# Acciorocketships/mrs-gym

Hardware: NVIDIA B200
Metric: agent-steps/sec (higher is better)
Workload: dtype f32

## Files before the change

### include/mrs_b200.h

```cpp
#ifndef MRS_B200_H
#define MRS_B200_H

#include <stddef.h>

#ifdef __cplusplus
extern "C" {
#endif

#define MRS_ABI_VERSION 5
#define MRS_STATE_PLANES 13
#define MRS_CTRL_PLANES 18
#define MRS_STATS_SLOTS 8
#define MRS_SCRATCH_PLANES 7
#define MRS_SCRATCH_PAIR_SPLITS 32
#define MRS_SYNC_WORDS 8208
#define MRS_COMM_MAX_WORLD 16
#define MRS_COMM_HANDLE_BYTES 64

typedef enum {
    MRS_SET_TARGET_VEL = 0,
    MRS_SET_TARGET_POS = 1,
    MRS_SET_TARGET_ACCEL = 2,
    MRS_SET_FORCE = 3,
    MRS_SET_TARGET_ORI = 4,
    MRS_SET_CONTROL = 5,
    MRS_SET_SPEEDS = 6,
    MRS_NO_ACTION = 7
} MrsActionType;

typedef enum {
    MRS_X_NONE = 0,
    MRS_X_POS_VEL = 1,
    MRS_X_FULL = 2
} MrsStateLayout;

typedef enum {
    MRS_OK = 0,
    MRS_ERR_ARG = -1,
    MRS_ERR_CUDA = -2,
    MRS_ERR_UNSUPPORTED = -3
} MrsError;

#define MRS_STATUS_NAN_ACTION 1u
#define MRS_STATUS_NONFINITE 2u
#define MRS_STATUS_CONTACT_OVERFLOW 16u
#define MRS_STATUS_SYNC_TIMEOUT 8u
#define MRS_STATUS_COMM_TIMEOUT 4u
#define MRS_STATUS_NEIGHBOR_OVERFLOW 32u

#define MRS_STAT_AGENT_CONTACTS 0
#define MRS_STAT_GROUND_CONTACTS 1
#define MRS_STAT_NONFINITE 2
#define MRS_STAT_NAN_ACTIONS 3
#define MRS_STAT_CONTACT_CHUNKS 4
#define MRS_STAT_SOLVER_SWEEPS 5
#define MRS_STAT_NEIGHBOR_OVERFLOW 6

typedef struct {
    float mass, ixx, iyy, izz;
    float kf, km, arm;
    float gnd_eff_coeff, prop_radius, gnd_hclip;
    float drag_xy, drag_z;
    float dw1, dw2, dw3;
    float prop_x[4], prop_y[4];
    float pos_p, pos_i, pos_d;
    float vel_p, vel_i, vel_d;
    float ori_p[3], ori_i[3], ori_d[3];
    float min_pwm, max_pwm, pwm2rpm_a, pwm2rpm_b;
    float ctrl_dt, ctrl_gravity;
    float mix_ainv[16];
    float mix_a[16];
    float nnls_tab[16 * 16];
} MrsQuadParams;

typedef struct {
    float mass;
    float inertia[3];
    float lin_damping, ang_damping;
    float max_coord_vel;
    int gyro;
    float ang_motion_threshold;
    float erp2, slop, contact_margin;
    float mu_ground, ground_z;
    float col_radius, col_halfheight, col_margin;
    int ground_contact, agent_contact;
    float agent_radius;
    float contact_radius;
    float mu_agent;
    int solver_iters;
    float solver_tol;
} MrsPhysicsParams;

typedef struct {
    int E, N, K, L;
    int action_type;
    int state_layout;
    float dt, gravity;
    float comm_range;
// ... 106 lines not shown
```

### mrs-gym_b200/csrc/mrs_step.cuh

```cuda
#pragma once
#include "mrs_common.cuh"
#include "mrs_contact_env.cuh"

namespace mrs {


__device__ __forceinline__ float* plane_ptr(float* p0, unsigned S, int pl) {
    return reinterpret_cast<float*>(reinterpret_cast<char*>(p0) + (unsigned long long)S * (unsigned)(pl * 4));
}
__device__ __forceinline__ const float* plane_ptr(const float* p0, unsigned S, int pl) {
    return reinterpret_cast<const float*>(reinterpret_cast<const char*>(p0) + (unsigned long long)S * (unsigned)(pl * 4));
}

template <int MODE, int GT>
static __device__ __noinline__ void chunk_step_contact(const MrsConfig* cptr, const Derived* dptr, const MrsBuffers* bptr,
                                                       const StepArgs* aptr, int G_in, int chunk, int t0, int T, unsigned lane_mask,
                                                       float4* wpos, unsigned* sh_events) {
    const MrsConfig& c = *cptr;
    const Derived& d = *dptr;
    const MrsBuffers& b = *bptr;
    const StepArgs& a = *aptr;
    const int lane = threadIdx.x & 31;
    const int G = GT ? GT : G_in;
    const int N = GT ? GT : c.N, E = c.E;
// ... 87 lines not shown
                v[0] += dv[0]; v[1] += dv[1]; v[2] += dv[2];
                worst = fmaxf(worst, wr);
            }
        };
        for (int it = 0; it < cp.solver_iters; ++it) {
            worst = 0.f;
            if (alive && g.act) worst = ground_sweep(cp, g, lam_g, fl, v, wb);
            if constexpr (kStaticRounds) {
#pragma unroll
                for (int r = 0; r < kRoundsMax; ++r)
                    if ((ract >> r) & 1u) do_round(r, lam_p + 3 * r);
            } else {
                for (unsigned m = ract; m; m &= m - 1u) {
                    const int r = __ffs(m) - 1;
                    do_round(r, lam_p + 3 * r);
                }
            }
            if (alive) ++n_sweeps;
            for (int o = G >> 1; o > 0; o >>= 1) worst = fmaxf(worst, __shfl_xor_sync(kFull32, worst, o));
            alive = alive && !(worst < cp.solver_tol);
            if (!__any_sync(kFull32, alive)) break;
        }
        st.vx = v[0]; st.vy = v[1]; st.vz = v[2];
        st.wx = R[0] * wb[0] + R[1] * wb[1] + R[2] * wb[2];
        st.wy = R[3] * wb[0] + R[4] * wb[1] + R[5] * wb[2];
        st.wz = R[6] * wb[0] + R[7] * wb[1] + R[8] * wb[2];
        if ((lam_g[0] + lam_g[1]) + (lam_g[2] + lam_g[3]) > 0.f) ++n_ground;
        if constexpr (kStaticRounds) {
#pragma unroll
            for (int r = 0; r < kRoundsMax; ++r)
                if (((ract >> r) & 1u) && lam_p[3 * r] > 0.f) ++n_agent_rows;
        } else {
            for (unsigned m = ract; m; m &= m - 1u)
                if (lam_p[3 * (__ffs(m) - 1)] > 0.f) ++n_agent_rows;
        }
    }
    integrate(c, d, st);
    if (!agent_finite(st)) status |= MRS_STATUS_NONFINITE;
    if (a.X0 && mine) write_X(a.X0 - (long long)t * a.xstride, c.state_layout, s, st);
    if (a.A0) {
        float* Arow = a.A0 - (long long)t * a.astride + (size_t)s * N;
        __syncwarp();
        wpos[lane] = make_float4(st.px, st.py, st.pz, 0.f);
        __syncwarp();
        if (mine) {
            for (int j = 0; j < N; ++j) {
                const float4 pj = wpos[gb + j];
                const float hit = d.comm_inf ? 1.f : adjacency_pair(st.px, st.py, st.pz, pj.x, pj.y, pj.z, d.s_max);
                MRS_TAPE_ST(Arow + j, (j == ai) ? 0.f : hit);
            }
        }
        __syncwarp();
    }
    if (!mine) { status = 0; n_agent_rows = 0; n_ground = 0; n_sweeps = 0; }
    {
        const unsigned any_status = __reduce_or_sync(kFull32, status);
        const unsigned sum_rows = __reduce_add_sync(kFull32, n_agent_rows);
        const unsigned sum_gnd = __reduce_add_sync(kFull32, n_ground);
        const unsigned max_sw = __reduce_max_sync(kFull32, n_sweeps);
        if (lane == 0) {
            if (any_status) atomicOr(&sh_events[0], any_status);
            if (sum_rows) atomicAdd(&sh_events[1], sum_rows);
            if (sum_gnd) atomicAdd(&sh_events[2], sum_gnd);
            if (any_status & MRS_STATUS_NONFINITE) atomicAdd(&sh_events[3], 1u);
            if (any_status & MRS_STATUS_NAN_ACTION) atomicAdd(&sh_events[4], 1u);
            if (max_sw) atomicAdd(&sh_events[6], max_sw);
        }
    }
  }
    if (mine) {
        store_agent(b.state, S, s, st);
        store_ctrl<MODE>(b.ctrl, S, s, k);
    }
}

template <int MODE, int GT> __host__ __device__ constexpr int group_warp_smem_bytes() {
#ifdef MRS_EXP_OLDSMEM
    return 1024 + ((MRS_PREFETCH && GT != 0) ? mode_stage_floats<MODE>() * 4 : 0);
#else
    return 512 + ((MRS_PREFETCH && GT != 0) ? mode_stage_floats<MODE>() * 4 : 0);
#endif
}

constexpr int kSyncCount = 8, kSyncQueue = 16, kSyncQueueLen = 1024, kSyncQueues = 8;
#ifndef MRS_DEFAULT_CPS
#define MRS_DEFAULT_CPS 4
#endif
static_assert(kSyncQueue + kSyncQueues * kSyncQueueLen <= MRS_SYNC_WORDS, "sync buffer layout");

template <int MODE, int GT, int WPB, bool BAKED, bool MANY>
__global__ void __launch_bounds__(WPB * 32, WPB == 4 ? ModeTraits<MODE>::minb : (4 * ModeTraits<MODE>::minb) / WPB)
#ifdef MRS_EXP_NOGC
step_group_kernel(const __grid_constant__ MrsConfig c_in, const __grid_constant__ Derived d_in, const MrsBuffers b,
                  const StepArgs a) {
#else
step_group_kernel(const __grid_constant__ MrsConfig c_in, const __grid_constant__ Derived d_in,
                  const __grid_constant__ MrsBuffers b, const __grid_constant__ StepArgs a) {
#endif
    MrsConfig c_bk;
    Derived d_bk;
    if constexpr (BAKED) baked_fill(c_bk, d_bk, c_in, d_in);
    const MrsConfig& c = BAKED ? c_bk : c_in;
    const Derived& d = BAKED ? d_bk : d_in;
    extern __shared__ __align__(16) unsigned char smem_raw[];
    constexpr bool kFull = GT != 0;
    constexpr bool kStage = MRS_PREFETCH && kFull;
    constexpr int kWarpBytes = group_warp_smem_bytes<MODE, GT>();
    __shared__ int sh_counter, sh_hi, sh_range, sh_lo, sh_pull;
    __shared__ unsigned sh_epoch;
    __shared__ unsigned sh_events[7];
    const int lane = threadIdx.x & 31, wib = threadIdx.x >> 5;
    unsigned char* wbase = smem_raw + wib * kWarpBytes;
    float4* wpos = reinterpret_cast<float4*>(wbase);
#ifdef MRS_EXP_OLDSMEM
    float* stage = reinterpret_cast<float*>(wbase + 1024);
#else
    float* stage = reinterpret_cast<float*>(wbase + 512);
#endif
    const int G = GT ? GT : a.G;
    const int N = GT ? GT : c.N;
    const int E = c.E;
    const int gpw = 32 / G;
    const int ai = lane & (G - 1);
    const int gb = lane - ai;
    const unsigned S = (unsigned)E * (unsigned)N;
    const int wtotal = gridDim.x * WPB;
    const MrsPhysicsParams& ph = c.phys;
    const bool pair_contact = ph.agent_contact && N > 1;

    constexpr bool kLocal = WPB > 4;
    constexpr bool kHand = kLocal && MRS_PREFETCH && GT != 0 && !MANY;
    const int T = MANY ? a.T : 1;
    const int gw = blockIdx.x * WPB + wib;
    if (threadIdx.x < 7) sh_events[threadIdx.x] = 0u;
    if (threadIdx.x == 7) sh_pull = 0;
    const int role = kHand ? a.role : 0;
    if (role == 2) {
        asm volatile("griddepcontrol.launch_dependents;");
        if (threadIdx.x == 0) {
            const unsigned long long* q = b.sync + kSyncQueue + ((a.seq - 1) & (kSyncQueues - 1)) * kSyncQueueLen + blockIdx.x;
            const unsigned long long* q3 = b.sync + kSyncQueue + ((a.seq - 3) & (kSyncQueues - 1)) * kSyncQueueLen + (gridDim.x - 1);
#ifdef MRS_EXP_NOBOUND
            const bool bound = false;
#else
            const bool bound = a.seq >= 3;
#endif
            unsigned long long e = ld_acquire_gpu_u64(q), e3 = bound ? ld_acquire_gpu_u64(q3) : 0ull, t0 = 0;
            unsigned epoch = (unsigned)ld_acquire_gpu_u64(b.sync);
            auto pending = [&]() {
                const unsigned long long tag = (unsigned long long)epoch << 16;
                return (e >> 16) != (tag | (unsigned)a.seq) || (bound && (e3 >> 16) != (tag | (unsigned)(a.seq - 2)));
            };
            while (pending()) {
                if (t0 == 0) t0 = global_ns();
                else if (global_ns() - t0 > 2000000000ull) {
                    if (b.status) atomicOr(b.status, MRS_STATUS_SYNC_TIMEOUT);
                    asm volatile("griddepcontrol.wait;" ::: "memory");
                    e = blockIdx.x;
                    break;
                }
                e = ld_acquire_gpu_u64(q);
                if (bound) e3 = ld_acquire_gpu_u64(q3);
                epoch = (unsigned)ld_acquire_gpu_u64(b.sync);
            }
            if (blockIdx.x == 0) atomicExch(b.sync + kSyncCount + ((a.seq + 4) & (kSyncQueues - 1)), 0ull);
            sh_range = (int)(e & 0xffffull);
            sh_epoch = epoch;
        }
    } else {
        if (role == 0) asm volatile("griddepcontrol.launch_dependents;");
        asm volatile("griddepcontrol.wait;" ::: "memory");
        if (threadIdx.x == 0) sh_range = blockIdx.x;
        if (role == 1) {
            if (blockIdx.x == 0 && threadIdx.x == 0) {
#pragma unroll
                for (int q = 0; q < kSyncQueues; ++q) atomicExch(b.sync + kSyncCount + q, 0ull);
                atomicAdd(b.sync, 1ull);
                __threadfence();
            }
            __syncthreads();
            asm volatile("griddepcontrol.launch_dependents;");
        }
    }
    if (threadIdx.x == 0) {
        const int nwork = a.nchunks - a.chunk_lo;
        const int r = sh_range;
        sh_counter = sh_lo = a.chunk_lo + (int)(((long long)r * nwork) / gridDim.x);
        sh_hi = a.chunk_lo + (int)(((long long)(r + 1) * nwork) / gridDim.x);
    }
    unsigned* parked = reinterpret_cast<unsigned*>(smem_raw + WPB * kWarpBytes);
    for (int i = threadIdx.x; i < a.slow_slots; i += WPB * 32) parked[i] = 0xffffffffu;
    __syncthreads();
    auto draw = [&]() -> int {
        int v = 0;
        asm volatile("{\n .reg .pred p;\n elect.sync _|p, 0xffffffff;\n @p atom.shared.add.u32 %0, [%1], 1;\n}"
                     : "+r"(v) : "r"((unsigned)__cvta_generic_to_shared(&sh_counter)) : "memory");
        return v;
    };
    const int chunk_hi = sh_hi;
    auto claim = [&](int v) -> int { return (v < chunk_hi) ? v : -1; };
    constexpr int kNC = mode_nctrl<MODE>();
    constexpr int kA = ModeTraits<MODE>::A;
    constexpr int kActBeg = 96, kActEnd = kActBeg + 8 * kA;
    constexpr int kP12Beg = kActEnd, kP12End = kP12Beg + 8;
    constexpr int kCtlBeg = kP12End, kCtlEnd = kCtlBeg + 8 * kNC;
    constexpr int kPieces = kCtlEnd;
    static_assert(kPieces * 4 == mode_stage_floats<MODE>(), "stage layout");
    const unsigned lane_el = (unsigned)(lane >> 3) * S + (unsigned)(lane & 7) * 4u;
    auto prefetch = [&](int chunk) {
        const unsigned s0 = (unsigned)chunk * 32u;
#pragma unroll
        for (int i = 0; i < (kPieces + 31) / 32; ++i) {
            const int q = lane + 32 * i;
            const int lo = 32 * i, hi = 32 * i + 31;
            if (hi < kActBeg) {
                cp_async16(stage + 4 * q, b.state + (lane_el + s0 + (unsigned)(4 * i) * S));
            } else {
                if (lo < kActEnd && hi >= kActBeg && (lo >= kActBeg || q >= kActBeg) && (hi < kActEnd || q < kActEnd))
                    cp_async16(stage + 4 * q, a.actions + (s0 * (unsigned)kA + (unsigned)(q - kActBeg) * 4u));
                if (lo < kP12End && hi >= kP12Beg && (lo >= kP12Beg || q >= kP12Beg) && (hi < kP12End || q < kP12End))
                    cp_async16(stage + 4 * q, b.state + (12u * S + s0 + (unsigned)(q - kP12Beg) * 4u));
                if (kNC > 0 && lo < kCtlEnd && hi >= kCtlBeg && (lo >= kCtlBeg || q >= kCtlBeg) && (hi < kCtlEnd || q < kCtlEnd)) {
                    const int cq = q - kCtlBeg;
                    cp_async16(stage + 4 * q, b.ctrl + ((unsigned)mode_ctrl_plane<MODE>(cq >> 3) * S + s0 + (unsigned)(cq & 7) * 4u));
                }
            }
        }
        cp_async_commit();
    };
#ifdef MRS_TRACE
    unsigned long long* trace = reinterpret_cast<unsigned long long*>(b.scratch) + (size_t)gw * 8;
    unsigned long long* agg = reinterpret_cast<unsigned long long*>(b.scratch) + (size_t)8192 * 8 + (size_t)a.slot_x * 4;
    int trace_i = 0;
    auto stamp = [&]() {
        unsigned long long tns;
        asm volatile("mov.u64 %0, %%globaltimer;" : "=l"(tns));
        if (lane == 0 && trace_i < 8) trace[trace_i] = tns;
        if (threadIdx.x == 0 && trace_i == 0) atomicMin(agg + 0, tns);
        if (threadIdx.x == 0 && trace_i == 1) atomicMax(agg + 1, tns);
        ++trace_i;
    };
    auto stamp_end = [&]() {
        unsigned long long tns;
        asm volatile("mov.u64 %0, %%globaltimer;" : "=l"(tns));
        if (threadIdx.x == 0) { atomicMax(agg + 2, tns); atomicMin(agg + 3, tns); }
    };
    stamp();
#endif
#ifdef MRS_TRACE
    stamp();
#endif
    int chunk, chunk_next;
    if (kLocal) {
        chunk = claim(__shfl_sync(kFull32, draw(), 0));
        chunk_next = chunk >= 0 ? claim(__shfl_sync(kFull32, draw(), 0)) : -1;
    } else {
        chunk = a.chunk_lo + gw;
        chunk_next = chunk + wtotal;
        if (chunk >= a.nchunks) chunk = -1;
        if (chunk_next >= a.nchunks) chunk_next = -1;
    }
    if (kStage && chunk >= 0) prefetch(chunk);
    const int rounds_static = kLocal ? 0 : (a.nchunks - a.chunk_lo + wtotal - 1) / wtotal;
    int round_i = 0, my_parked = 0;
    while (chunk >= 0) {
        const int ticket = (kLocal && chunk_next >= 0) ? draw() : -1;
        const int e = chunk * gpw + (lane / G);
        const bool valid = kFull ? true : ((e < E) && (ai < N));
        const unsigned s = kFull ? (unsigned)chunk * 32u + (unsigned)lane
                                 : (valid ? (unsigned)e * (unsigned)N + (unsigned)ai : 0u);
        Agent st;
        Ctrl k;
        float4 act0 = make_float4(0.f, 0.f, 0.f, 0.f);
        if constexpr (kStage) {
            cp_async_wait_all();
            __syncwarp();
            st.px = stage[0 * 32 + lane]; st.py = stage[1 * 32 + lane]; st.pz = stage[2 * 32 + lane];
            st.qx = stage[3 * 32 + lane]; st.qy = stage[4 * 32 + lane]; st.qz = stage[5 * 32 + lane];
            st.qw = stage[6 * 32 + lane];
            st.vx = stage[7 * 32 + lane]; st.vy = stage[8 * 32 + lane]; st.vz = stage[9 * 32 + lane];
            st.wx = stage[10 * 32 + lane]; st.wy = stage[11 * 32 + lane]; st.wz = stage[4 * kP12Beg + lane];
            const float* cs = stage + 4 * kCtlBeg + lane;
            if constexpr (ModeTraits<MODE>::io) {
#pragma unroll
                for (int i = 0; i < 3; ++i) k.io[i] = cs[i * 32];
            }
            if constexpr (ModeTraits<MODE>::ip) {
#pragma unroll
                for (int i = 0; i < 3; ++i) k.ip[i] = cs[(3 + i) * 32];
            }
            if constexpr (ModeTraits<MODE>::vel) {
#pragma unroll
                for (int i = 0; i < 3; ++i) {
                    k.iv[i] = cs[(3 + i) * 32]; k.lve[i] = cs[(6 + i) * 32];
                    k.dve[i] = cs[(9 + i) * 32]; k.ltv[i] = cs[(12 + i) * 32];
                }
            }
            const float* as = stage + 4 * kActBeg + kA * lane;
            if constexpr (kA == 4) act0 = *reinterpret_cast<const float4*>(as);
            if constexpr (kA == 3) act0 = make_float4(as[0], as[1], as[2], 0.f);
            __syncwarp();
            if (chunk_next >= 0) prefetch(chunk_next);
        } else if (valid) {
            load_agent(b.state, S, s, st);
            load_ctrl<MODE>(b.ctrl, S, s, k);
        } else {
            dummy_agent(st);
#pragma unroll
            for (int i = 0; i < 3; ++i) k.io[i] = k.ip[i] = k.iv[i] = k.lve[i] = k.dve[i] = k.ltv[i] = 0.f;
        }
        float* Xs = a.X0;
        float* As = a.A0;
        if (!kStage) {
            float tmp[4] = {0.f, 0.f, 0.f, 0.f};
            if (valid) (void)load_action<MODE>(a.actions, (size_t)s, tmp);
            act0 = make_float4(tmp[0], tmp[1], tmp[2], tmp[3]);
        }
        bool state_stored = false;
        for (int t = 0; t < T; ++t, Xs -= a.xstride, As -= a.astride) {
            unsigned status = 0;
            unsigned n_agent_rows = 0, n_ground = 0;
            float rpm[4];
            float act[4] = {act0.x, act0.y, act0.z, act0.w};
            if (kA > 0 && valid && (isnan(act0.x) || isnan(act0.y) || isnan(act0.z) || (kA == 4 && isnan(act0.w))))
                status |= MRS_STATUS_NAN_ACTION;
            if (MANY && t + 1 < T && valid) {
                float tmp[4];
                (void)load_action<MODE>(a.actions, (size_t)(t + 1) * S + s, tmp);
                act0 = make_float4(tmp[0], tmp[1], tmp[2], tmp[3]);
            }

#ifdef MRS_EXP_COPYONLY
            st.px += act[0] * 1e-12f;
            if (false) {
#else
            {
#endif
            float dw = 0.f;
// ... 103 lines not shown
                            MRS_TAPE_ST(reinterpret_cast<float4*>(Arow0 + col), make_float4(v0[0], v0[1], v0[2], v0[3]));
                            MRS_TAPE_ST(reinterpret_cast<float4*>(Arow0 + GT + col), make_float4(v1[0], v1[1], v1[2], v1[3]));
                        }
                    } else if (valid) {
                        for (int j = 0; j < N; ++j) Arow[j] = (j == ai) ? 0.f : 1.f;
                    }
                } else {
                    __syncwarp();
                    wpos[lane] = make_float4(st.px, st.py, st.pz, 0.f);
                    __syncwarp();
                    if constexpr (GT != 0) {
                        const int h = lane & 1;
                        const float4 r0 = wpos[lane & ~1], r1 = wpos[lane | 1];
                        float* Arow0 = As + (size_t)(s & ~1u) * GT;
                        const int d0 = (ai & ~1) - 4 * h;
#pragma unroll
                        for (int qq = 0; qq < GT / 8; ++qq) {
                            const int col = 8 * qq + 4 * h;
                            float4 pj[4];
#pragma unroll
                            for (int u = 0; u < 4; ++u) pj[u] = wpos[gb + col + u];
                            float v0[4], v1[4];
#pragma unroll
                            for (int u = 0; u < 4; ++u) {
                                const float h0 = adjacency_pair(r0.x, r0.y, r0.z, pj[u].x, pj[u].y, pj[u].z, d.s_max);
                                const float h1 = adjacency_pair(r1.x, r1.y, r1.z, pj[u].x, pj[u].y, pj[u].z, d.s_max);
                                v0[u] = (8 * qq + u == d0) ? 0.f : h0;
                                v1[u] = (8 * qq + u == d0 + 1) ? 0.f : h1;
                            }
                            MRS_TAPE_ST(reinterpret_cast<float4*>(Arow0 + col), make_float4(v0[0], v0[1], v0[2], v0[3]));
                            MRS_TAPE_ST(reinterpret_cast<float4*>(Arow0 + GT + col), make_float4(v1[0], v1[1], v1[2], v1[3]));
                        }
                    } else if (valid) {
                        if ((N & 3) == 0) {
#pragma unroll 2
                            for (int j = 0; j < N; j += 4) {
                                float4 pj[4];
#pragma unroll
                                for (int u = 0; u < 4; ++u) pj[u] = wpos[gb + j + u];
                                float v[4];
#pragma unroll
                                for (int u = 0; u < 4; ++u) {
                                    const float hit = adjacency_pair(st.px, st.py, st.pz, pj[u].x, pj[u].y, pj[u].z, d.s_max);
                                    v[u] = (j + u == ai) ? 0.f : hit;
                                }
                                MRS_TAPE_ST(reinterpret_cast<float4*>(Arow + j), make_float4(v[0], v[1], v[2], v[3]));
                            }
                        } else {
                            for (int j = 0; j < N; ++j) {
                                const float4 pj = wpos[gb + j];
                                const float hit = adjacency_pair(st.px, st.py, st.pz, pj.x, pj.y, pj.z, d.s_max);
                                Arow[j] = (j == ai) ? 0.f : hit;
                            }
                        }
                    }
                }
            }
            }
            if (!valid || state_stored) { status = 0; n_agent_rows = 0; n_ground = 0; }
            if (__reduce_or_sync(kFull32, status | n_agent_rows | n_ground)) {
                const unsigned any_status = __reduce_or_sync(kFull32, status);
                const unsigned sum_rows = __reduce_add_sync(kFull32, n_agent_rows);
                const unsigned sum_gnd = __reduce_add_sync(kFull32, n_ground);
                if (lane == 0) {
                    if (any_status) atomicOr(&sh_events[0], any_status);
                    if (sum_rows) atomicAdd(&sh_events[1], sum_rows);
                    if (sum_gnd) atomicAdd(&sh_events[2], sum_gnd);
                    if (any_status & MRS_STATUS_NONFINITE) atomicAdd(&sh_events[3], 1u);
                    if (any_status & MRS_STATUS_NAN_ACTION) atomicAdd(&sh_events[4], 1u);
                }
            }
        }

        if (valid && !state_stored) {
            float* p0 = b.state + s;
            *plane_ptr(p0, S, 0) = st.px; *plane_ptr(p0, S, 1) = st.py; *plane_ptr(p0, S, 2) = st.pz;
            *plane_ptr(p0, S, 3) = st.qx; *plane_ptr(p0, S, 4) = st.qy; *plane_ptr(p0, S, 5) = st.qz;
            *plane_ptr(p0, S, 6) = st.qw;
            *plane_ptr(p0, S, 7) = st.vx; *plane_ptr(p0, S, 8) = st.vy; *plane_ptr(p0, S, 9) = st.vz;
            *plane_ptr(p0, S, 10) = st.wx; *plane_ptr(p0, S, 11) = st.wy; *plane_ptr(p0, S, 12) = st.wz;
            store_ctrl<MODE>(b.ctrl, S, s, k);
        }
#ifdef MRS_TRACE
        stamp();
#endif
        chunk = chunk_next;
        ++round_i;
        if (kLocal) {
            chunk_next = (chunk >= 0) ? claim(__shfl_sync(kFull32, ticket, 0)) : -1;
        } else {
            chunk_next = (chunk >= 0 && chunk + wtotal < a.nchunks) ? chunk + wtotal : -1;
        }
    }
#ifndef MRS_EXP_NOCALL
    if (__syncthreads_or(my_parked)) {
        const int n_slots = kLocal ? sh_hi - sh_lo : WPB * rounds_static;
        for (;;) {
            int i = 0;
            if (lane == 0) i = atomicAdd(&sh_pull, 1);
            i = __shfl_sync(kFull32, i, 0);
            if (i >= n_slots) break;
            const unsigned e = parked[i];
            if (e == 0xffffffffu) continue;
            const int w = (int)(e >> 16);
            const int pc = kLocal ? sh_lo + i : a.chunk_lo + blockIdx.x * WPB + w + (i - w * rounds_static) * wtotal;
            chunk_step_contact<MODE, GT>(&c_in, &d_in, &b, &a, GT ? GT : a.G, pc, (int)(e & 0xffffu), T, kFull32, wpos, sh_events);
        }
    }
#endif
    __syncthreads();
    if (threadIdx.x == 0) {
        if (sh_events[0] && b.status) atomicOr(b.status, sh_events[0]);
        if (b.stats) {
            if (sh_events[1]) atomicAdd(b.stats + MRS_STAT_AGENT_CONTACTS, (unsigned long long)sh_events[1]);
            if (sh_events[2]) atomicAdd(b.stats + MRS_STAT_GROUND_CONTACTS, (unsigned long long)sh_events[2]);
            if (sh_events[3]) atomicAdd(b.stats + MRS_STAT_NONFINITE, (unsigned long long)sh_events[3]);
            if (sh_events[4]) atomicAdd(b.stats + MRS_STAT_NAN_ACTIONS, (unsigned long long)sh_events[4]);
            if (sh_events[5]) atomicAdd(b.stats + MRS_STAT_CONTACT_CHUNKS, (unsigned long long)sh_events[5]);
            if (sh_events[6]) atomicAdd(b.stats + MRS_STAT_SOLVER_SWEEPS, (unsigned long long)sh_events[6]);
        }
        if (role != 0) {
            __threadfence();
            const unsigned epoch = (role == 1) ? (unsigned)ld_acquire_gpu_u64(b.sync) : sh_epoch;
            const int q = a.seq & (kSyncQueues - 1);
            const unsigned long long j = atomicAdd(b.sync + kSyncCount + q, 1ull);
            st_release_gpu_u64(b.sync + kSyncQueue + q * kSyncQueueLen + (int)(j & (kSyncQueueLen - 1)),
                               ((unsigned long long)epoch << 32) | ((unsigned long long)(a.seq + 1) << 16) | (unsigned)sh_range);
        }
    }
#ifdef MRS_TRACE
    stamp_end();
#endif
}

template <int LPA>
__device__ __forceinline__ float group_sum(float v) {
#pragma unroll
    for (int o = LPA / 2; o > 0; o >>= 1) v += __shfl_xor_sync(kFull32, v, o);
    return v;
}

template <int MODE>
__device__ __forceinline__ void agent_pre(const MrsConfig& c, const Derived& d, const MrsBuffers& b,
                                          const float* __restrict__ actions, unsigned S, unsigned s, float dw, bool near) {
    Agent st;
    Ctrl k;
    load_agent(b.state, S, s, st);
    load_ctrl<MODE>(b.ctrl, S, s, k);
    const float pix = st.px, piy = st.py, piz = st.pz;
    float act[4];
    unsigned status = 0;
    if (load_action<MODE>(actions, s, act)) status |= MRS_STATUS_NAN_ACTION;
    float R[9], rpm[4];
    quat_to_mat(st, R);
    if (status) {
        rpm[0] = rpm[1] = rpm[2] = rpm[3] = 0.f;
        dw = 0.f;
    } else {
        action_to_rpm<MODE>(c, c.quad, d, st, R, act, k, rpm);
    }
    apply_wrench<MODE != MRS_NO_ACTION>(c, d, st, R, rpm, dw);
    float* sc = b.scratch;
    sc[0 * (size_t)S + s] = st.vx; sc[1 * (size_t)S + s] = st.vy; sc[2 * (size_t)S + s] = st.vz;
    sc[3 * (size_t)S + s] = pix; sc[4 * (size_t)S + s] = piy; sc[5 * (size_t)S + s] = piz;
    sc[6 * (size_t)S + s] = near ? 1.f : 0.f;
    b.state[10 * (size_t)S + s] = st.wx; b.state[11 * (size_t)S + s] = st.wy; b.state[12 * (size_t)S + s] = st.wz;
    store_ctrl<MODE>(b.ctrl, S, s, k);
    if (b.rpm && MODE != MRS_NO_ACTION) {
#pragma unroll
        for (int i = 0; i < 4; ++i) b.rpm[i * (size_t)S + s] = rpm[i];
    }
    if (status && b.status) {
        atomicOr(b.status, status);
        if (b.stats) atomicAdd(b.stats + MRS_STAT_NAN_ACTIONS, 1ull);
    }
}

template <int MODE, int LPA>
__global__ void __launch_bounds__(kBlock)
step_pre_kernel(const __grid_constant__ MrsConfig c, const __grid_constant__ Derived d, const MrsBuffers b,
                const float* __restrict__ actions) {
    pdl_enter();
    const int N = c.N;
    const unsigned S = (unsigned)c.E * (unsigned)N;
    const unsigned gid = (blockIdx.x * kBlock + threadIdx.x) / LPA;
    const int l = threadIdx.x & (LPA - 1);
    const bool valid = gid < S;
    const unsigned s = valid ? gid : 0u;
    const unsigned env0 = (s / (unsigned)N) * (unsigned)N;
    const int ai = (int)(s - env0);
    const float* __restrict__ px = b.state + 0 * (size_t)S + env0;
    const float* __restrict__ py = b.state + 1 * (size_t)S + env0;
    const float* __restrict__ pz = b.state + 2 * (size_t)S + env0;
    const float pix = px[ai], piy = py[ai], piz = pz[ai];
    float dw = 0.f;
    bool near = false;
    const bool pair_contact = c.phys.agent_contact && N > 1;
    if (MODE != MRS_NO_ACTION || pair_contact) {
        for (int j0 = 0; j0 < N; j0 += 4 * LPA) {
            float dxy2[4], rz[4];
            bool live[4], any_live = false;
#pragma unroll
            for (int u = 0; u < 4; ++u) {
                const int j = j0 + u * LPA + l;
                const bool in = j < N;
                const int jj = in ? j : ai;
                const float rx = px[jj] - pix, ry = py[jj] - piy;
                rz[u] = pz[jj] - piz;
                dxy2[u] = rx * rx + ry * ry;
                const bool other = in && j != ai;
                const float beta = c.quad.dw2 * rz[u] + c.quad.dw3;
                live[u] = MODE != MRS_NO_ACTION && other && rz[u] > 0.f && dxy2[u] < 100.f &&
                          !(dxy2[u] > 208.f * beta * beta);
                any_live = any_live || live[u];
// ... 226 lines not shown
    const unsigned env0 = env * (unsigned)N;
    const int i = it * kBlock + threadIdx.x;
    const bool valid = i < N;
    const float* __restrict__ px = b.state + 0 * (size_t)S + env0;
    const float* __restrict__ py = b.state + 1 * (size_t)S + env0;
    const float* __restrict__ pz = b.state + 2 * (size_t)S + env0;
    const float pix = valid ? px[i] : 0.f, piy = valid ? py[i] : 0.f, piz = valid ? pz[i] : 3.0e18f;
    const bool pair_contact = c.phys.agent_contact && N > 1;
    const unsigned lim_m1 = __float_as_uint(d.lim2) - 1u;
    float dw = 0.f;
    bool near = false;
    __shared__ float tile_zmax[kBlock / 32];
    float wz_min = valid ? piz : 3.0e38f;
#pragma unroll
    for (int o = 16; o > 0; o >>= 1) wz_min = fminf(wz_min, __shfl_xor_sync(kFull32, wz_min, o));
    const float z_skip = wz_min - sqrtf(d.lim2);
    const int jbeg = js * jw, jend = min(jbeg + jw, N);
    for (int j0 = jbeg; j0 < jend; j0 += kBlock) {
        const int jj = j0 + threadIdx.x;
        const float4 mine = (jj < jend) ? make_float4(px[jj], py[jj], pz[jj], 0.f) : make_float4(3.0e18f, 0.f, -3.0e18f, 0.f);
        float zm = mine.z;
#pragma unroll
        for (int o = 16; o > 0; o >>= 1) zm = fmaxf(zm, __shfl_xor_sync(kFull32, zm, o));
        __syncthreads();
        tile[threadIdx.x] = mine;
        if ((threadIdx.x & 31) == 0) tile_zmax[threadIdx.x >> 5] = zm;
        __syncthreads();
        const float tz = fmaxf(fmaxf(tile_zmax[0], tile_zmax[1]), fmaxf(tile_zmax[2], tile_zmax[3]));
        if (tz < z_skip) continue;
#pragma unroll 2
        for (int jl = 0; jl < kBlock; jl += 4) {
            float dxy2[4], rz[4];
            bool live[4], any_live = false;
#pragma unroll
            for (int u = 0; u < 4; ++u) {
                const float4 pj = tile[jl + u];
                const float rx = pj.x - pix, ry = pj.y - piy;
                rz[u] = pj.z - piz;
                dxy2[u] = rx * rx + ry * ry;
                const float d2 = dxy2[u] + rz[u] * rz[u];
                near = near || (__float_as_uint(d2) - 1u < lim_m1);
                const float beta = c.quad.dw2 * rz[u] + c.quad.dw3;
                live[u] = MODE != MRS_NO_ACTION && rz[u] > 0.f && dxy2[u] < 100.f && !(dxy2[u] > 208.f * beta * beta);
                any_live = any_live || live[u];
            }
            if (MODE != MRS_NO_ACTION && __any_sync(kFull32, any_live)) {
#pragma unroll
                for (int u = 0; u < 4; ++u) {
                    const float f = downwash_pair(c.quad, d, dxy2[u], rz[u]);
                    dw += live[u] ? f : 0.f;
                }
            }
        }
    }
    if (!valid) return;
    const unsigned s = env0 + (unsigned)i;
    b.scratch[(size_t)(kPairPlane0 + js) * S + s] = dw;
    b.scratch[(size_t)(kPairPlane0 + nsplit + js) * S + s] = (near && pair_contact) ? 1.f : 0.f;
}

template <int MODE>
__global__ void __launch_bounds__(kBlock)
agent_pre_kernel(const __grid_constant__ MrsConfig c, const __grid_constant__ Derived d, const MrsBuffers b,
                 const float* __restrict__ actions, int nsplit) {
    pdl_enter();
    const unsigned S = (unsigned)c.E * (unsigned)c.N;
    const unsigned s = blockIdx.x * kBlock + threadIdx.x;
    if (s >= S) return;
    float dw = 0.f, fl = 0.f;
    for (int j0 = 0; j0 < nsplit; j0 += 8) {
        float pd[8], pf[8];
#pragma unroll
        for (int u = 0; u < 8; ++u) {
            const bool in = j0 + u < nsplit;
            pd[u] = in ? b.scratch[(size_t)(kPairPlane0 + j0 + u) * S + s] : 0.f;
            pf[u] = in ? b.scratch[(size_t)(kPairPlane0 + nsplit + j0 + u) * S + s] : 0.f;
        }
#pragma unroll
        for (int u = 0; u < 8; ++u) { dw += pd[u]; fl += pf[u]; }
    }
    agent_pre<MODE>(c, d, b, actions, S, s, dw, fl != 0.f);
}

template <int MODE, int GT, int WPB, bool BAKED, bool MANY>
static int launch_group_wpb(const MrsConfig& c, const Derived& d, const MrsBuffers& b, const StepArgs& a_in, long long blocks,
                            bool pdl, cudaStream_t st) {
    StepArgs a = a_in;
    const long long nwork = a.nchunks - a.chunk_lo;
    a.slow_slots = (WPB > 4) ? (int)((nwork + blocks - 1) / blocks) + 1
                             : WPB * (int)((nwork + blocks * WPB - 1) / (blocks * WPB));
    const size_t smem = (size_t)WPB * group_warp_smem_bytes<MODE, GT>() + (((size_t)a.slow_slots * 4 + 15) & ~(size_t)15);
    if (smem > 200 * 1024) return MRS_ERR_UNSUPPORTED;
    static size_t configured[64] = {};
    int dev = 0;
    if (cudaGetDevice(&dev) != cudaSuccess || dev < 0 || dev >= 64) return MRS_ERR_CUDA;
    if (smem > 48 * 1024 && smem > configured[dev]) {
        if (cudaFuncSetAttribute(step_group_kernel<MODE, GT, WPB, BAKED, MANY>, cudaFuncAttributeMaxDynamicSharedMemorySize, (int)smem) !=
            cudaSuccess)
            return MRS_ERR_CUDA;
        configured[dev] = smem;
    }
    cudaLaunchConfig_t lc = {};
    lc.gridDim = dim3((unsigned)blocks);
    lc.blockDim = dim3(WPB * 32);
    lc.dynamicSmemBytes = smem;
    lc.stream = st;
    cudaLaunchAttribute attr[1];
    attr[0].id = cudaLaunchAttributeProgrammaticStreamSerialization;
    attr[0].val.programmaticStreamSerializationAllowed = 1;
    lc.attrs = attr;
    lc.numAttrs = pdl ? 1 : 0;
    if (cudaLaunchKernelEx(&lc, step_group_kernel<MODE, GT, WPB, BAKED, MANY>, c, d, b, a) != cudaSuccess) {
        (void)cudaGetLastError();
        return MRS_ERR_CUDA;
    }
    return last_error();
}

template <int MODE, int GT, int WPB>
static int launch_group_variant(const MrsConfig& c, const Derived& d, const MrsBuffers& b, const StepArgs& a, long long blocks,
                                bool pdl, bool baked, cudaStream_t st) {
    if (a.T > 1)
        return baked ? launch_group_wpb<MODE, GT, WPB, true, true>(c, d, b, a, blocks, pdl, st)
                     : launch_group_wpb<MODE, GT, WPB, false, true>(c, d, b, a, blocks, pdl, st);
    return baked ? launch_group_wpb<MODE, GT, WPB, true, false>(c, d, b, a, blocks, pdl, st)
                 : launch_group_wpb<MODE, GT, WPB, false, false>(c, d, b, a, blocks, pdl, st);
}

template <int MODE, int GT>
static int launch_group(const MrsConfig& c, const Derived& d, const MrsBuffers& b, StepArgs a, cudaStream_t st) {
    constexpr int kBig = 4 * ModeTraits<MODE>::minb;
    const int sms = sm_count();
    if (sms <= 0) return MRS_ERR_CUDA;
    static const int use_pdl = env_int("MRS_B200_PDL", 1);
    static const int use_big = env_int("MRS_B200_BIGCTA", 1);
    static const int use_hand = env_int("MRS_B200_HANDOVER", 1);
    static const int use_baked = env_int("MRS_B200_BAKED", 1);
    const bool baked = use_baked && config_is_baked(c, d);
    const int nwork = a.nchunks - a.chunk_lo;
    if (use_big && nwork > 2 * sms * kBig) {
        if (a.T > 1) {
            a.role = 0;
            return launch_group_variant<MODE, GT, kBig>(c, d, b, a, sms, use_pdl != 0, baked, st);
        }
        static const int cps = env_int("MRS_B200_CPS", MRS_DEFAULT_CPS);
        if (!(use_hand && use_pdl && b.sync && GT != 0 && sms * cps <= kSyncQueueLen)) a.role = 0;
#ifdef MRS_CPS_VARIANTS
        if (cps == 1) return launch_group_variant<MODE, GT, kBig>(c, d, b, a, sms, use_pdl != 0, baked, st);
        if (cps == 2) return launch_group_variant<MODE, GT, kBig / 2>(c, d, b, a, 2 * sms, use_pdl != 0, baked, st);
#endif
        return launch_group_variant<MODE, GT, kBig / MRS_DEFAULT_CPS>(c, d, b, a, MRS_DEFAULT_CPS * sms, use_pdl != 0, baked, st);
    }
    a.role = 0;
    const long long need = ((long long)nwork + 3) / 4;
    const long long cap = (long long)sms * ModeTraits<MODE>::minb;
    const long long blocks = need < cap ? need : cap;
    const bool pdl = use_pdl && need >= cap;
    return launch_group_variant<MODE, GT, 4>(c, d, b, a, blocks, pdl, baked, st);
}

template <int MODE, int LPA>
static int launch_wide_lpa(const MrsConfig& c, const Derived& d, const MrsBuffers& b, const StepArgs& a, cudaStream_t st) {
    const size_t S = (size_t)c.E * c.N;
    constexpr int A = ModeTraits<MODE>::A;
    const unsigned blocks = (unsigned)((S * LPA + kBlock - 1) / kBlock);
    SideLane* L = (b.A_tape && a.T > 1) ? side_lane() : nullptr;
    int jw = 0, nsplit = 0;
    if (LPA > 32) pair_split(c.E, c.N, &jw, &nsplit);
    for (int t = 0; t < a.T; ++t) {
        const float* act_t = a.actions ? a.actions + (size_t)t * S * A : nullptr;
        if constexpr (LPA > 32) {
            const int itiles = (c.N + kBlock - 1) / kBlock;
            if (int rc = launch_pdl(true, pair_tile_kernel<MODE>, dim3((unsigned)((long long)itiles * nsplit * c.E)), kBlock, 0, st, c, d,
                                    b, jw, nsplit))
                return rc;
            if (int rc = launch_pdl(true, agent_pre_kernel<MODE>, dim3((unsigned)((S + kBlock - 1) / kBlock)), kBlock, 0, st, c, d, b,
                                    act_t, nsplit))
                return rc;
        } else {
            if (int rc = launch_pdl(false, step_pre_kernel<MODE, LPA>, dim3(blocks), kBlock, 0, st, c, d, b, act_t)) return rc;
        }
        if (int rc = launch_contact_env(c, d, b, LPA > 32, st)) return rc;
        if (L && t > 0 && cudaStreamWaitEvent(st, L->adj_done, 0) != cudaSuccess) return MRS_ERR_CUDA;
        if (int rc = launch_step_post(c, d, b, a.slot_x - t, LPA > 32, st)) return rc;
        if (b.A_tape) {
            cudaStream_t as = st;
            if (L) {
                if (cudaEventRecord(L->posted, st) != cudaSuccess) return MRS_ERR_CUDA;
                if (cudaStreamWaitEvent(L->s, L->posted, 0) != cudaSuccess) return MRS_ERR_CUDA;
                as = L->s;
            }
            const int rc = launch_adjacency(b.state, S, 1, b.A_tape + (size_t)(a.slot_a - t) * S * c.N, c.E, c.N, d.s_max,
                                            d.comm_inf, as);
            if (rc) return rc;
            if (L && cudaEventRecord(L->adj_done, L->s) != cudaSuccess) return MRS_ERR_CUDA;
        }
    }
    if (L && cudaStreamWaitEvent(st, L->adj_done, 0) != cudaSuccess) return MRS_ERR_CUDA;
    return last_error();
}

template <int MODE>
static int launch_mid(const MrsConfig& c, const Derived& d, const MrsBuffers& b, const StepArgs& a, cudaStream_t st) {
    const size_t S = (size_t)c.E * c.N;
    constexpr int A = ModeTraits<MODE>::A;
    const unsigned blocks = (unsigned)((S + kBlock - 1) / kBlock);
    SideLane* L = (b.A_tape && a.T > 1) ? side_lane() : nullptr;
    for (int t = 0; t < a.T; ++t) {
        const float* act_t = a.actions ? a.actions + (size_t)t * S * A : nullptr;
        if (int rc = launch_pdl(false, step_mid_pre_kernel<MODE>, dim3(blocks), kBlock, 0, st, c, d, b, act_t)) return rc;
        if (int rc = launch_contact_env(c, d, b, false, st)) return rc;
        if (L && t > 0 && cudaStreamWaitEvent(st, L->adj_done, 0) != cudaSuccess) return MRS_ERR_CUDA;
        if (int rc = launch_step_post(c, d, b, a.slot_x - t, false, st)) return rc;
        if (b.A_tape) {
            cudaStream_t as = st;
            if (L) {
                if (cudaEventRecord(L->posted, st) != cudaSuccess) return MRS_ERR_CUDA;
                if (cudaStreamWaitEvent(L->s, L->posted, 0) != cudaSuccess) return MRS_ERR_CUDA;
                as = L->s;
            }
            const int rc = launch_adjacency(b.state, S, 1, b.A_tape + (size_t)(a.slot_a - t) * S * c.N, c.E, c.N, d.s_max,
                                            d.comm_inf, as);
            if (rc) return rc;
            if (L && cudaEventRecord(L->adj_done, L->s) != cudaSuccess) return MRS_ERR_CUDA;
        }
    }
    if (L && cudaStreamWaitEvent(st, L->adj_done, 0) != cudaSuccess) return MRS_ERR_CUDA;
    return last_error();
}

template <int MODE>
static int launch_env_fused(const MrsConfig& c, const Derived& d, const MrsBuffers& b, const StepArgs& a, cudaStream_t st) {
    const size_t S = (size_t)c.E * c.N;
    constexpr int A = ModeTraits<MODE>::A;
    const unsigned threads = (unsigned)((c.N + 31) / 32 * 32);
    const size_t smem = contact_env_smem((int)threads, c.N);
    for (int t = 0; t < a.T; ++t) {
        const float* act_t = a.actions ? a.actions + (size_t)t * S * A : nullptr;
        float* A_slice = b.A_tape ? b.A_tape + (size_t)(a.slot_a - t) * S * c.N : nullptr;
        if (int rc = launch_pdl(true, step_env_kernel<MODE>, dim3((unsigned)c.E), threads, smem, st, c, d, b, act_t, a.slot_x - t,
                                A_slice))
// ... 61 lines not shown
```

### mrs-gym_b200/mrsgym_b200/_abi.py

```python
from __future__ import annotations

import ctypes as C
import os

_HERE = os.path.dirname(os.path.abspath(__file__))
LIB_PATH = os.environ.get('MRS_B200_LIB') or os.path.join(_HERE, 'libmrs_b200.so')

ABI_VERSION = 5
STATE_PLANES = 13
CTRL_PLANES = 18
STATS_SLOTS = 8
SCRATCH_PLANES = 7
SYNC_WORDS = 8208

ACTION_TYPES = dict(set_target_vel=0, set_target_pos=1, set_target_accel=2, set_force=3,
                    set_target_ori=4, set_control=5, set_speeds=6)
NO_ACTION = 7
ACTION_DIMS = {0: 3, 1: 3, 2: 3, 3: 3, 4: 3, 5: 4, 6: 4, 7: 0}

X_NONE, X_POS_VEL, X_FULL = 0, 1, 2
STATE_DIMS = {X_NONE: 0, X_POS_VEL: 6, X_FULL: 13}

STATUS_NAN_ACTION = 1
STATUS_NONFINITE = 2
STATUS_COMM_TIMEOUT = 4
STATUS_SYNC_TIMEOUT = 8
STATUS_CONTACT_OVERFLOW = 16
STATUS_NEIGHBOR_OVERFLOW = 32
COMM_MAX_WORLD = 16
COMM_HANDLE_BYTES = 64
STAT_NAMES = ('agent_contact_rows', 'ground_contacts', 'nonfinite', 'nan_actions', 'contact_chunks', 'solver_sweeps',
              'neighbor_overflow')

f = C.c_float


class MrsQuadParams(C.Structure):
    _fields_ = [('mass', f), ('ixx', f), ('iyy', f), ('izz', f),
                ('kf', f), ('km', f), ('arm', f),
                ('gnd_eff_coeff', f), ('prop_radius', f), ('gnd_hclip', f),
                ('drag_xy', f), ('drag_z', f),
                ('dw1', f), ('dw2', f), ('dw3', f),
                ('prop_x', f * 4), ('prop_y', f * 4),
                ('pos_p', f), ('pos_i', f), ('pos_d', f),
                ('vel_p', f), ('vel_i', f), ('vel_d', f),
                ('ori_p', f * 3), ('ori_i', f * 3), ('ori_d', f * 3),
                ('min_pwm', f), ('max_pwm', f), ('pwm2rpm_a', f), ('pwm2rpm_b', f),
                ('ctrl_dt', f), ('ctrl_gravity', f),
                ('mix_ainv', f * 16), ('mix_a', f * 16), ('nnls_tab', f * 256)]


class MrsPhysicsParams(C.Structure):
    _fields_ = [('mass', f), ('inertia', f * 3),
                ('lin_damping', f), ('ang_damping', f), ('max_coord_vel', f),
                ('gyro', C.c_int), ('ang_motion_threshold', f),
                ('erp2', f), ('slop', f), ('contact_margin', f),
                ('mu_ground', f), ('ground_z', f),
                ('col_radius', f), ('col_halfheight', f), ('col_margin', f),
                ('ground_contact', C.c_int), ('agent_contact', C.c_int),
                ('agent_radius', f), ('contact_radius', f), ('mu_agent', f), ('solver_iters', C.c_int),
                ('solver_tol', f)]


class MrsConfig(C.Structure):
    _fields_ = [('E', C.c_int), ('N', C.c_int), ('K', C.c_int), ('L', C.c_int),
                ('action_type', C.c_int), ('state_layout', C.c_int),
                ('dt', f), ('gravity', f), ('comm_range', f),
                ('quad', MrsQuadParams), ('phys', MrsPhysicsParams)]


class MrsBuffers(C.Structure):
    _fields_ = [('state', C.c_void_p), ('ctrl', C.c_void_p), ('rpm', C.c_void_p),
                ('X_tape', C.c_void_p), ('A_tape', C.c_void_p), ('scratch', C.c_void_p),
                ('status', C.c_void_p), ('stats', C.c_void_p), ('sync', C.c_void_p)]


class MrsAutoResetArgs(C.Structure):
    _fields_ = [('seed', C.c_ulonglong), ('env_offset', C.c_ulonglong),
                ('z_lo', f), ('z_hi', f), ('xy_radius', f), ('xy_sigma', f), ('yaw_lo', f), ('yaw_hi', f),
                ('max_rounds', C.c_int), ('episode_length', C.c_int), ('max_timesteps', C.c_int)]


class MrsError(RuntimeError):
    pass


_SIGNATURES = {
    'mrs_abi_version': (C.c_int, []),
    'mrs_strerror': (C.c_char_p, [C.c_int]),
    'mrs_state_dim': (C.c_int, [C.c_int]),
    'mrs_action_dim': (C.c_int, [C.c_int]),
    'mrs_scratch_planes': (C.c_int, [C.c_int, C.c_int]),
    'mrs_sizeof_config': (C.c_size_t, []),
    'mrs_sizeof_buffers': (C.c_size_t, []),
    'mrs_default_config': (C.c_int, [C.POINTER(MrsConfig)]),
    'mrs_config_is_baked': (C.c_int, [C.POINTER(MrsConfig)]),
# ... 68 lines not shown
```

Measured before the change: 34.09 billion.

## Use single-warp CTAs for the range path with sharded sync counters

For large workloads the range path now launches one-warp blocks, with many more blocks per SM, instead of blocks sized by a fixed CPS default. Shared-memory chunk claiming becomes a per-warp local counter, and syncthreads becomes syncwarp. Cross-launch completion queues shard their atomic counters into 32 groups with padded strides, which reduces contention now that there are far more blocks. This enlarges the sync buffer and queue length, and adds scheduling overhead from the higher block count.

```diff
diff --git a/include/mrs_b200.h b/include/mrs_b200.h
--- a/include/mrs_b200.h
+++ b/include/mrs_b200.h
@@ -13,7 +13,7 @@
 #define MRS_STATS_SLOTS 8
 #define MRS_SCRATCH_PLANES 7
 #define MRS_SCRATCH_PAIR_SPLITS 32
-#define MRS_SYNC_WORDS 8208
+#define MRS_SYNC_WORDS 69648
 #define MRS_COMM_MAX_WORLD 16
 #define MRS_COMM_HANDLE_BYTES 64
 
diff --git a/mrs-gym_b200/csrc/mrs_step.cuh b/mrs-gym_b200/csrc/mrs_step.cuh
--- a/mrs-gym_b200/csrc/mrs_step.cuh
+++ b/mrs-gym_b200/csrc/mrs_step.cuh
@@ -193,14 +193,17 @@
 #endif
 }
 
-constexpr int kSyncCount = 8, kSyncQueue = 16, kSyncQueueLen = 1024, kSyncQueues = 8;
-#ifndef MRS_DEFAULT_CPS
-#define MRS_DEFAULT_CPS 4
-#endif
+constexpr int kSyncGroups = 32, kSyncCtrStride = 16, kSyncQueues = 8;
+constexpr int kSyncCount = 8, kSyncQueue = kSyncCount + kSyncQueues * kSyncGroups * kSyncCtrStride + 8;
+constexpr int kSyncQueueLen = 8192;
+__device__ __forceinline__ unsigned long long* sync_counter(unsigned long long* sync, int q, int g) {
+    return sync + kSyncCount + (q * kSyncGroups + g) * kSyncCtrStride;
+}
+static_assert(kSyncQueue == 4112, "sync buffer layout (comment above)");
 static_assert(kSyncQueue + kSyncQueues * kSyncQueueLen <= MRS_SYNC_WORDS, "sync buffer layout");
 
-template <int MODE, int GT, int WPB, bool BAKED, bool MANY>
-__global__ void __launch_bounds__(WPB * 32, WPB == 4 ? ModeTraits<MODE>::minb : (4 * ModeTraits<MODE>::minb) / WPB)
+template <int MODE, int GT, int WPB, bool RANGE, bool BAKED, bool MANY>
+__global__ void __launch_bounds__(WPB * 32, RANGE ? (4 * ModeTraits<MODE>::minb) / WPB : ModeTraits<MODE>::minb)
 #ifdef MRS_EXP_NOGC
 step_group_kernel(const __grid_constant__ MrsConfig c_in, const __grid_constant__ Derived d_in, const MrsBuffers b,
                   const StepArgs a) {
@@ -239,10 +242,18 @@
     const MrsPhysicsParams& ph = c.phys;
     const bool pair_contact = ph.agent_contact && N > 1;
 
-    constexpr bool kLocal = WPB > 4;
+    constexpr bool kLocal = RANGE;
     constexpr bool kHand = kLocal && MRS_PREFETCH && GT != 0 && !MANY;
+    auto cta_sync = [&]() {
+        if constexpr (WPB == 1) __syncwarp();
+        else __syncthreads();
+    };
     const int T = MANY ? a.T : 1;
     const int gw = blockIdx.x * WPB + wib;
+#ifdef MRS_TRACE
+    unsigned long long trace_entry;
+    asm volatile("mov.u64 %0, %%globaltimer;" : "=l"(trace_entry));
+#endif
     if (threadIdx.x < 7) sh_events[threadIdx.x] = 0u;
     if (threadIdx.x == 7) sh_pull = 0;
     const int role = kHand ? a.role : 0;
@@ -250,7 +261,9 @@
         asm volatile("griddepcontrol.launch_dependents;");
         if (threadIdx.x == 0) {
             const unsigned long long* q = b.sync + kSyncQueue + ((a.seq - 1) & (kSyncQueues - 1)) * kSyncQueueLen + blockIdx.x;
-            const unsigned long long* q3 = b.sync + kSyncQueue + ((a.seq - 3) & (kSyncQueues - 1)) * kSyncQueueLen + (gridDim.x - 1);
+            const int grp = (int)(blockIdx.x % kSyncGroups);
+            const unsigned long long* q3 = b.sync + kSyncQueue + ((a.seq - 3) & (kSyncQueues - 1)) * kSyncQueueLen +
+                                           grp + kSyncGroups * ((gridDim.x - 1 - grp) / kSyncGroups);
 #ifdef MRS_EXP_NOBOUND
             const bool bound = false;
 #else
@@ -274,7 +287,7 @@
                 if (bound) e3 = ld_acquire_gpu_u64(q3);
                 epoch = (unsigned)ld_acquire_gpu_u64(b.sync);
             }
-            if (blockIdx.x == 0) atomicExch(b.sync + kSyncCount + ((a.seq + 4) & (kSyncQueues - 1)), 0ull);
+            if (blockIdx.x < kSyncGroups) atomicExch(sync_counter(b.sync, (a.seq + 4) & (kSyncQueues - 1), blockIdx.x), 0ull);
             sh_range = (int)(e & 0xffffull);
             sh_epoch = epoch;
         }
@@ -285,11 +298,12 @@
         if (role == 1) {
             if (blockIdx.x == 0 && threadIdx.x == 0) {
 #pragma unroll
-                for (int q = 0; q < kSyncQueues; ++q) atomicExch(b.sync + kSyncCount + q, 0ull);
+                for (int q = 0; q < kSyncQueues; ++q)
+                    for (int g = 0; g < kSyncGroups; ++g) atomicExch(sync_counter(b.sync, q, g), 0ull);
                 atomicAdd(b.sync, 1ull);
                 __threadfence();
             }
-            __syncthreads();
+            cta_sync();
             asm volatile("griddepcontrol.launch_dependents;");
         }
     }
@@ -301,13 +315,16 @@
     }
     unsigned* parked = reinterpret_cast<unsigned*>(smem_raw + WPB * kWarpBytes);
     for (int i = threadIdx.x; i < a.slow_slots; i += WPB * 32) parked[i] = 0xffffffffu;
-    __syncthreads();
+    cta_sync();
+    int next_chunk = sh_lo;
     auto draw = [&]() -> int {
+        if constexpr (WPB == 1) return next_chunk++;
         int v = 0;
         asm volatile("{\n .reg .pred p;\n elect.sync _|p, 0xffffffff;\n @p atom.shared.add.u32 %0, [%1], 1;\n}"
                      : "+r"(v) : "r"((unsigned)__cvta_generic_to_shared(&sh_counter)) : "memory");
         return v;
     };
+    auto from_lane0 = [&](int v) -> int { return WPB == 1 ? v : __shfl_sync(kFull32, v, 0); };
     const int chunk_hi = sh_hi;
     auto claim = [&](int v) -> int { return (v < chunk_hi) ? v : -1; };
     constexpr int kNC = mode_nctrl<MODE>();
@@ -342,29 +359,20 @@
 #ifdef MRS_TRACE
     unsigned long long* trace = reinterpret_cast<unsigned long long*>(b.scratch) + (size_t)gw * 8;
     unsigned long long* agg = reinterpret_cast<unsigned long long*>(b.scratch) + (size_t)8192 * 8 + (size_t)a.slot_x * 4;
-    int trace_i = 0;
-    auto stamp = [&]() {
+    auto stamp = [&](int i) {
         unsigned long long tns;
         asm volatile("mov.u64 %0, %%globaltimer;" : "=l"(tns));
-        if (lane == 0 && trace_i < 8) trace[trace_i] = tns;
-        if (threadIdx.x == 0 && trace_i == 0) atomicMin(agg + 0, tns);
-        if (threadIdx.x == 0 && trace_i == 1) atomicMax(agg + 1, tns);
-        ++trace_i;
+        if (lane == 0) trace[i] = tns;
+        if (threadIdx.x == 0 && i == 1) { atomicMin(agg + 0, tns); atomicMax(agg + 1, tns); }
+        if (threadIdx.x == 0 && i == 7) { atomicMax(agg + 2, tns); atomicMin(agg + 3, tns); }
     };
-    auto stamp_end = [&]() {
-        unsigned long long tns;
-        asm volatile("mov.u64 %0, %%globaltimer;" : "=l"(tns));
-        if (threadIdx.x == 0) { atomicMax(agg + 2, tns); atomicMin(agg + 3, tns); }
-    };
-    stamp();
-#endif
-#ifdef MRS_TRACE
-    stamp();
+    if (lane == 0) trace[0] = trace_entry;
+    stamp(1);
 #endif
     int chunk, chunk_next;
     if (kLocal) {
-        chunk = claim(__shfl_sync(kFull32, draw(), 0));
-        chunk_next = chunk >= 0 ? claim(__shfl_sync(kFull32, draw(), 0)) : -1;
+        chunk = claim(from_lane0(draw()));
+        chunk_next = chunk >= 0 ? claim(from_lane0(draw())) : -1;
     } else {
         chunk = a.chunk_lo + gw;
         chunk_next = chunk + wtotal;
@@ -634,18 +642,28 @@
             store_ctrl<MODE>(b.ctrl, S, s, k);
         }
 #ifdef MRS_TRACE
-        stamp();
+        if (round_i < 4) stamp(2 + round_i);
 #endif
         chunk = chunk_next;
         ++round_i;
         if (kLocal) {
-            chunk_next = (chunk >= 0) ? claim(__shfl_sync(kFull32, ticket, 0)) : -1;
+            chunk_next = (chunk >= 0) ? claim(from_lane0(ticket)) : -1;
         } else {
             chunk_next = (chunk >= 0 && chunk + wtotal < a.nchunks) ? chunk + wtotal : -1;
         }
     }
+#ifdef MRS_TRACE
+    stamp(6);
+#endif
 #ifndef MRS_EXP_NOCALL
-    if (__syncthreads_or(my_parked)) {
+    bool any_parked;
+    if constexpr (WPB == 1) {
+        __syncwarp();
+        any_parked = __any_sync(kFull32, my_parked);
+    } else {
+        any_parked = __syncthreads_or(my_parked);
+    }
+    if (any_parked) {
         const int n_slots = kLocal ? sh_hi - sh_lo : WPB * rounds_static;
         for (;;) {
             int i = 0;
@@ -660,7 +678,7 @@
         }
     }
 #endif
-    __syncthreads();
+    cta_sync();
     if (threadIdx.x == 0) {
         if (sh_events[0] && b.status) atomicOr(b.status, sh_events[0]);
         if (b.stats) {
@@ -675,13 +693,14 @@
             __threadfence();
             const unsigned epoch = (role == 1) ? (unsigned)ld_acquire_gpu_u64(b.sync) : sh_epoch;
             const int q = a.seq & (kSyncQueues - 1);
-            const unsigned long long j = atomicAdd(b.sync + kSyncCount + q, 1ull);
-            st_release_gpu_u64(b.sync + kSyncQueue + q * kSyncQueueLen + (int)(j & (kSyncQueueLen - 1)),
+            const int grp = (int)(blockIdx.x % kSyncGroups);
+            const unsigned long long j = atomicAdd(sync_counter(b.sync, q, grp), 1ull);
+            st_release_gpu_u64(b.sync + kSyncQueue + q * kSyncQueueLen + (int)((grp + kSyncGroups * j) & (kSyncQueueLen - 1)),
                                ((unsigned long long)epoch << 32) | ((unsigned long long)(a.seq + 1) << 16) | (unsigned)sh_range);
         }
     }
 #ifdef MRS_TRACE
-    stamp_end();
+    stamp(7);
 #endif
 }
 
@@ -1074,12 +1093,12 @@
     agent_pre<MODE>(c, d, b, actions, S, s, dw, fl != 0.f);
 }
 
-template <int MODE, int GT, int WPB, bool BAKED, bool MANY>
+template <int MODE, int GT, int WPB, bool RANGE, bool BAKED, bool MANY>
 static int launch_group_wpb(const MrsConfig& c, const Derived& d, const MrsBuffers& b, const StepArgs& a_in, long long blocks,
                             bool pdl, cudaStream_t st) {
     StepArgs a = a_in;
     const long long nwork = a.nchunks - a.chunk_lo;
-    a.slow_slots = (WPB > 4) ? (int)((nwork + blocks - 1) / blocks) + 1
+    a.slow_slots = RANGE ? (int)((nwork + blocks - 1) / blocks) + 1
                              : WPB * (int)((nwork + blocks * WPB - 1) / (blocks * WPB));
     const size_t smem = (size_t)WPB * group_warp_smem_bytes<MODE, GT>() + (((size_t)a.slow_slots * 4 + 15) & ~(size_t)15);
     if (smem > 200 * 1024) return MRS_ERR_UNSUPPORTED;
@@ -1087,7 +1106,7 @@
     int dev = 0;
     if (cudaGetDevice(&dev) != cudaSuccess || dev < 0 || dev >= 64) return MRS_ERR_CUDA;
     if (smem > 48 * 1024 && smem > configured[dev]) {
-        if (cudaFuncSetAttribute(step_group_kernel<MODE, GT, WPB, BAKED, MANY>, cudaFuncAttributeMaxDynamicSharedMemorySize, (int)smem) !=
+        if (cudaFuncSetAttribute(step_group_kernel<MODE, GT, WPB, RANGE, BAKED, MANY>, cudaFuncAttributeMaxDynamicSharedMemorySize, (int)smem) !=
             cudaSuccess)
             return MRS_ERR_CUDA;
         configured[dev] = smem;
@@ -1102,26 +1121,26 @@
     attr[0].val.programmaticStreamSerializationAllowed = 1;
     lc.attrs = attr;
     lc.numAttrs = pdl ? 1 : 0;
-    if (cudaLaunchKernelEx(&lc, step_group_kernel<MODE, GT, WPB, BAKED, MANY>, c, d, b, a) != cudaSuccess) {
+    if (cudaLaunchKernelEx(&lc, step_group_kernel<MODE, GT, WPB, RANGE, BAKED, MANY>, c, d, b, a) != cudaSuccess) {
         (void)cudaGetLastError();
         return MRS_ERR_CUDA;
     }
     return last_error();
 }
 
-template <int MODE, int GT, int WPB>
+template <int MODE, int GT, int WPB, bool RANGE>
 static int launch_group_variant(const MrsConfig& c, const Derived& d, const MrsBuffers& b, const StepArgs& a, long long blocks,
                                 bool pdl, bool baked, cudaStream_t st) {
     if (a.T > 1)
-        return baked ? launch_group_wpb<MODE, GT, WPB, true, true>(c, d, b, a, blocks, pdl, st)
-                     : launch_group_wpb<MODE, GT, WPB, false, true>(c, d, b, a, blocks, pdl, st);
-    return baked ? launch_group_wpb<MODE, GT, WPB, true, false>(c, d, b, a, blocks, pdl, st)
-                 : launch_group_wpb<MODE, GT, WPB, false, false>(c, d, b, a, blocks, pdl, st);
+        return baked ? launch_group_wpb<MODE, GT, WPB, RANGE, true, true>(c, d, b, a, blocks, pdl, st)
+                     : launch_group_wpb<MODE, GT, WPB, RANGE, false, true>(c, d, b, a, blocks, pdl, st);
+    return baked ? launch_group_wpb<MODE, GT, WPB, RANGE, true, false>(c, d, b, a, blocks, pdl, st)
+                 : launch_group_wpb<MODE, GT, WPB, RANGE, false, false>(c, d, b, a, blocks, pdl, st);
 }
 
 template <int MODE, int GT>
 static int launch_group(const MrsConfig& c, const Derived& d, const MrsBuffers& b, StepArgs a, cudaStream_t st) {
-    constexpr int kBig = 4 * ModeTraits<MODE>::minb;
+    constexpr int kSmWarps = 4 * ModeTraits<MODE>::minb;
     const int sms = sm_count();
     if (sms <= 0) return MRS_ERR_CUDA;
     static const int use_pdl = env_int("MRS_B200_PDL", 1);
@@ -1130,25 +1149,33 @@
     static const int use_baked = env_int("MRS_B200_BAKED", 1);
     const bool baked = use_baked && config_is_baked(c, d);
     const int nwork = a.nchunks - a.chunk_lo;
-    if (use_big && nwork > 2 * sms * kBig) {
+    if (use_big && nwork > 2 * sms * kSmWarps) {
         if (a.T > 1) {
             a.role = 0;
-            return launch_group_variant<MODE, GT, kBig>(c, d, b, a, sms, use_pdl != 0, baked, st);
-        }
-        static const int cps = env_int("MRS_B200_CPS", MRS_DEFAULT_CPS);
+            return launch_group_variant<MODE, GT, kSmWarps, true>(c, d, b, a, sms, use_pdl != 0, baked, st);
+        }
+        constexpr int kWpb = 1;
+        int cps = kSmWarps / kWpb;
+#ifdef MRS_CPS_VARIANTS
+        cps = env_int("MRS_B200_CPS", cps);
+#endif
         if (!(use_hand && use_pdl && b.sync && GT != 0 && sms * cps <= kSyncQueueLen)) a.role = 0;
 #ifdef MRS_CPS_VARIANTS
-        if (cps == 1) return launch_group_variant<MODE, GT, kBig>(c, d, b, a, sms, use_pdl != 0, baked, st);
-        if (cps == 2) return launch_group_variant<MODE, GT, kBig / 2>(c, d, b, a, 2 * sms, use_pdl != 0, baked, st);
-#endif
-        return launch_group_variant<MODE, GT, kBig / MRS_DEFAULT_CPS>(c, d, b, a, MRS_DEFAULT_CPS * sms, use_pdl != 0, baked, st);
+        constexpr int kMinb = ModeTraits<MODE>::minb;
+        if (cps == 4) return launch_group_variant<MODE, GT, kMinb, true>(c, d, b, a, 4ll * sms, use_pdl != 0, baked, st);
+        if (cps == kMinb) return launch_group_variant<MODE, GT, 4, true>(c, d, b, a, (long long)cps * sms, use_pdl != 0, baked, st);
+        if (cps == 2 * kMinb) return launch_group_variant<MODE, GT, 2, true>(c, d, b, a, (long long)cps * sms, use_pdl != 0, baked, st);
+        if (cps == 4 * kMinb) return launch_group_variant<MODE, GT, 1, true>(c, d, b, a, (long long)cps * sms, use_pdl != 0, baked, st);
+        return MRS_ERR_ARG;
+#endif
+        return launch_group_variant<MODE, GT, kWpb, true>(c, d, b, a, (long long)(kSmWarps / kWpb) * sms, use_pdl != 0, baked, st);
     }
     a.role = 0;
     const long long need = ((long long)nwork + 3) / 4;
     const long long cap = (long long)sms * ModeTraits<MODE>::minb;
     const long long blocks = need < cap ? need : cap;
     const bool pdl = use_pdl && need >= cap;
-    return launch_group_variant<MODE, GT, 4>(c, d, b, a, blocks, pdl, baked, st);
+    return launch_group_variant<MODE, GT, 4, false>(c, d, b, a, blocks, pdl, baked, st);
 }
 
 template <int MODE, int LPA>
diff --git a/mrs-gym_b200/mrsgym_b200/_abi.py b/mrs-gym_b200/mrsgym_b200/_abi.py
--- a/mrs-gym_b200/mrsgym_b200/_abi.py
+++ b/mrs-gym_b200/mrsgym_b200/_abi.py
@@ -11,7 +11,7 @@
 CTRL_PLANES = 18
 STATS_SLOTS = 8
 SCRATCH_PLANES = 7
-SYNC_WORDS = 8208
+SYNC_WORDS = 69648
 
 ACTION_TYPES = dict(set_target_vel=0, set_target_pos=1, set_target_accel=2, set_force=3,
                     set_target_ori=4, set_control=5, set_speeds=6)
```

After: 31.85 billion, median of 6. 6.6% lower.
